# pyannote/pyannote-video

Hardware: AMD Instinct MI355X
Metric: frames/sec end-to-end detect->embed->cluster, 1080p@25fps (higher is better)
Workload: dtype f32 (detector scores, embedder) / f64 (tracker, clustering) / u8 frames; an f16 screening pass with a proven error bound decides which windows the detector's exact f32 chain is evaluated for -- results identical to dense f32 scoring (`dense_scoring`)

## Files before the change

### pyannote-video_amd/csrc/detect.hip

```cpp
#include "detect_ml.h"
#include <algorithm>
#include <thread>
#include <cmath>
#include <cstdlib>

#define RESIZE_MAXS 22
struct RowTab { int32_t top, bottom; double tb, tb1, pad; };
struct ColTab { int32_t left, pad; double lr, lr1, pad2; };

template <int RS, int NSTRIP>
__global__ void __launch_bounds__(256) resize_rows_k(const uint8_t* const* __restrict__ in_ptrs, const uint8_t* __restrict__ in_base,
                                                     size_t in_stride, int in_rb, int ih, int iw, uint8_t* __restrict__ out,
                                                     size_t out_stride, int out_rb, int oh, int ow,
                                                     const RowTab* __restrict__ rows, const ColTab* __restrict__ cols)
{
    constexpr int MAXS = (RS == 16) ? RESIZE_MAXS : (RS * 5) / 4 + 3;
    __shared__ uint32_t s_rows[4][MAXS][64];
    __shared__ uint32_t s_out[4][64];
    const int lane = threadIdx.x & 63;
    const int wave = __builtin_amdgcn_readfirstlane(threadIdx.x >> 6);
    const int c0 = blockIdx.x * 256 + wave * 64;
    const int b = blockIdx.z;
    if (c0 >= ow) return;
    const int c = min(c0 + lane, ow - 1);
    const uint8_t* in = in_ptrs ? in_ptrs[b] : in_base + (size_t)b * in_stride;
    uint8_t* ob = out + (size_t)b * out_stride + (size_t)c0 * 3;
    const ColTab ct = cols[c];
    const int left = ct.left;
    const int left0 = __builtin_amdgcn_readfirstlane(left);
    const bool has_right = (left + 1 <= iw - 1);
    const double lr = ct.lr, lr1 = ct.lr1;
    const int seg_bytes = min(ow - c0, 64) * 3;
    const bool stores = (4 * lane < seg_bytes);
    const unsigned delta = (unsigned)((uintptr_t)in & 3u);
    const __amdgpu_buffer_rsrc_t rs = __builtin_amdgcn_make_buffer_rsrc((void*)((uintptr_t)in - delta), 0, (int)(delta + (unsigned)ih * (unsigned)in_rb), 0x00020000);
    const int lane4 = 4 * lane;
    int r0 = blockIdx.y * (RS * NSTRIP), r_end = 0, s_first = 0;
    unsigned win0 = 0;
    uint32_t t[MAXS];
    auto request = [&](int q0, int& sf, unsigned& w0) {
        const int qe = min(q0 + RS, oh);
        sf = rows[q0].top;
        const int nr = rows[qe - 1].bottom - sf + 1;
        w0 = delta + (unsigned)sf * (unsigned)in_rb + 3u * (unsigned)left0;
#pragma unroll
        for (int k = 0; k < MAXS; ++k) {
            t[k] = 0;
            if (k < nr) t[k] = __builtin_amdgcn_raw_buffer_load_b32(rs, lane4, (int)((w0 + (unsigned)k * (unsigned)in_rb) & ~3u), 0);
        }
    };
    request(r0, s_first, win0);
    const uint8_t* wl = reinterpret_cast<const uint8_t*>(&s_rows[wave][0][0]) + 3 * (left - left0);
    const uint8_t* wr = wl + (has_right ? 3 : 0);
    uint8_t* so = reinterpret_cast<uint8_t*>(&s_out[wave][0]) + 3 * lane;
    const uint32_t* sd = &s_out[wave][0] + lane;
    auto hblend = [&](int srow, double* hh) {
        const int k = srow - s_first;
        const unsigned off = 256u * (unsigned)k + ((win0 + (unsigned)k * (unsigned)in_rb) & 3u);
        typedef const volatile __attribute__((address_space(3))) uint8_t* lds_bytes;
        lds_bytes pl = (lds_bytes)(wl + off);
        lds_bytes pr = (lds_bytes)(wr + off);
        const uint32_t l0 = pl[0], l1 = pl[1], l2 = pl[2], q0 = pr[0], q1 = pr[1], q2 = pr[2];
        hh[0] = lr1 * (double)l0 + lr * (double)q0;
        hh[1] = lr1 * (double)l1 + lr * (double)q1;
        hh[2] = lr1 * (double)l2 + lr * (double)q2;
    };
    const __amdgpu_buffer_rsrc_t ro = __builtin_amdgcn_make_buffer_rsrc((void*)ob, 0, (int)((unsigned)oh * (unsigned)out_rb - 3u * (unsigned)c0), 0x00020000);
    const int st_off = stores ? lane4 : 0x7fffff00;
    auto emit = [&](int r, double tb, double tb1, const double* ht, const double* hb) {
#pragma unroll
        for (int k = 0; k < 3; ++k) {
            const double v = tb1 * ht[k] + tb * hb[k];
            so[k] = (uint8_t)(v + 0.5);
        }
        __builtin_amdgcn_wave_barrier();
        const uint32_t dw = *sd;
        __builtin_amdgcn_wave_barrier();
        __builtin_amdgcn_raw_buffer_store_b32(dw, ro, st_off, r * out_rb, 0);
    };
    int r = 0, srow = 0;
    double hA[3], hB[3];
    const __attribute__((address_space(4))) RowTab* crows = (const __attribute__((address_space(4))) RowTab*)rows;
    int top_r = 0;
    auto step = [&](const double* hc, double* hn) {
        const int ra = min(r, oh - 1), rb = min(r + 1, oh - 1), rc = min(r + 2, oh - 1);
        const double tbA = crows[ra].tb, tb1A = crows[ra].tb1, tbB = crows[rb].tb, tb1B = crows[rb].tb1;
        const int topB = crows[rb].top, topC = crows[rc].top;
        hblend(min(srow + 1, ih - 1), hn);
        if (top_r == srow) {
            emit(r, tbA, tb1A, hc, hn);
            ++r;
            top_r = topB;
            if (r < r_end && top_r == srow) {
                emit(r, tbB, tb1B, hc, hn);
                ++r;
                top_r = topC;
                while (r < r_end && top_r == srow) {
                    emit(r, crows[r].tb, crows[r].tb1, hc, hn);
                    ++r;
                    top_r = crows[min(r, oh - 1)].top;
                }
            }
        }
        ++srow;
    };
#pragma unroll 1
    for (int strip = 0; strip < NSTRIP; ++strip) {
#pragma unroll
        for (int k = 0; k < MAXS; ++k) s_rows[wave][k][lane] = t[k];
        __builtin_amdgcn_wave_barrier();
        r_end = min(r0 + RS, oh);
        const int q0 = r0 + RS;
        const bool more = (strip + 1 < NSTRIP) && (q0 < oh);
        int n_first = 0;
        unsigned n_win0 = 0;
        if (more) request(q0, n_first, n_win0);
        r = r0; srow = s_first; top_r = s_first;
        hblend(srow, hA);
        while (r < r_end) {
            step(hA, hB);
            if (r >= r_end) break;
            step(hB, hA);
        }
        if (!more) break;
        __builtin_amdgcn_wave_barrier();
        r0 = q0; s_first = n_first; win0 = n_win0;
    }
}

static std::vector<double> resize_coords(int n_in, int n_out)
{
    const double scale = (n_in - 1) / (double)std::max(n_out - 1, 1);
    const char* mode = getenv("PVF_RESIZE_COORDS");
    const bool accumulate = mode && strcmp(mode, "accumulate") == 0;
    PVF_REQUIRE(!mode || accumulate || strcmp(mode, "mul") == 0, "PVF_RESIZE_COORDS must be mul or accumulate");
    std::vector<double> v((size_t)n_out);
    double a = -scale;
    for (int i = 0; i < n_out; ++i) { a += scale; v[i] = accumulate ? a : i * scale; }
    return v;
}

static void fill_row_table(std::vector<RowTab>& t, int ih, int oh)
{
    const std::vector<double> ys = resize_coords(ih, oh);
    const size_t base = t.size();
    t.resize(base + oh);
    for (int r = 0; r < oh; ++r) {
        const double y = ys[r];
        RowTab& e = t[base + r];
        e.top = (int)std::floor(y);
        e.bottom = std::min(e.top + 1, ih - 1);
        e.tb = y - e.top;
        e.tb1 = 1 - e.tb;
        e.pad = 0;
    }
}

static void fill_col_table(std::vector<ColTab>& t, int iw, int ow)
{
    const std::vector<double> xs = resize_coords(iw, ow);
    const size_t base = t.size();
    t.resize(base + ow);
    for (int c = 0; c < ow; ++c) {
        ColTab& e = t[base + c];
        e.left = (int)std::floor(xs[c]);
        e.lr = xs[c] - e.left;
        e.lr1 = 1 - e.lr;
        e.pad = 0; e.pad2 = 0;
    }
}

static void launch_resize_rows(Ctx* c, const uint8_t* const* in_ptrs, const uint8_t* in_base, size_t in_stride, int in_rb, int ih, int iw,
                               uint8_t* out, size_t out_stride, int out_rb, int oh, int ow, int batch, const RowTab* d_rows, const ColTab* d_cols)
{
    const double x_scale = (iw - 1) / (double)std::max(ow - 1, 1);
    const double y_scale = (ih - 1) / (double)std::max(oh - 1, 1);
    constexpr int RS = 16;
    PVF_REQUIRE(x_scale <= 1.25 && y_scale <= 1.25 && (RS - 1) * y_scale + 3 <= RESIZE_MAXS, "resize_rows: scale outside the pyramid's range (2x up, 6/5 down)");
    PVF_REQUIRE(out_rb % 4 == 0 && out_stride % 4 == 0 && ((uintptr_t)out & 3) == 0 && out_rb >= (ow * 3 + 3) / 4 * 4, "resize: output rows must be 4-byte aligned");
    constexpr int NSTRIP = 2;
    static const int thin = getenv("PVF_RESIZE_THIN") ? atoi(getenv("PVF_RESIZE_THIN")) : 0;
    if (thin) {
        dim3 grid8((ow + 255) / 256, (oh + 8 * NSTRIP - 1) / (8 * NSTRIP), batch);
        hipLaunchKernelGGL((resize_rows_k<8, NSTRIP>), grid8, dim3(256), 0, c->det_stream, in_ptrs, in_base, in_stride, in_rb, ih, iw, out, out_stride, out_rb, oh, ow, d_rows, d_cols);
        return;
    }
    dim3 grid((ow + 255) / 256, (oh + RS * NSTRIP - 1) / (RS * NSTRIP), batch);
    hipLaunchKernelGGL((resize_rows_k<RS, NSTRIP>), grid, dim3(256), 0, c->det_stream, in_ptrs, in_base, in_stride, in_rb, ih, iw, out, out_stride, out_rb, oh, ow, d_rows, d_cols);
}

static void pyramid_up_dims(int ih, int iw, int* oh, int* ow)
{
    const double right = ((iw - 1) + 1.25) * 2.0;
    const double bottom = ((ih - 1) + 0.75) * 2.0;
    *ow = (int)std::floor(right + 0.5) + 1;
    *oh = (int)std::floor(bottom + 0.5) + 1;
}


static inline long iround(double v) { return (long)std::floor(v + 0.5); }
static void rect_down6(long r[4]) { const double ratio = (6 - 1.0) / 6; for (int i = 0; i < 4; ++i) r[i] = iround((r[i] - 0.3) * ratio + 0.3); }
static void rect_up6(long r[4]) { const double ratio = 6 / (6 - 1.0); for (int i = 0; i < 4; ++i) r[i] = iround((r[i] - 0.3) * ratio + 0.3); }
static void rect_down2i(long r[4])
{
    r[0] = iround(r[0] / 2.0 - 1.25); r[1] = iround(r[1] / 2.0 - 0.75);
    r[2] = iround(r[2] / 2.0 - 1.25); r[3] = iround(r[3] / 2.0 - 0.75);
}
static int detector_levels(int h, int w, const DetectorModel& m)
{
    long r[4] = {0, 0, w - 1, h - 1};
    int levels = 0;
    do { rect_down6(r); ++levels; } while ((r[2] - r[0] + 1) >= m.min_w && (r[3] - r[1] + 1) >= m.min_h && levels < m.max_levels);
    return levels;
}
static void fhog_to_image(long px, long py, int cell, int pad_r, int pad_c, long* ox, long* oy)
{
    long x = (px + 1 - (pad_c - 1) / 2) * cell + 1;
    long y = (py + 1 - (pad_r - 1) / 2) * cell + 1;
    x += (x >= 0) ? cell / 2 : -(cell / 2);
    y += (y >= 0) ? cell / 2 : -(cell / 2);
    *ox = x; *oy = y;
}

struct LevelDims { int h, w; };
static std::vector<LevelDims> level_schedule(int h, int w, int upsample, const DetectorModel& m, std::vector<LevelDims>* ups)
{
    int ch = h, cw = w;
    for (int u = 0; u < upsample; ++u) {
        int nh, nw;
        pyramid_up_dims(ch, cw, &nh, &nw);
        ch = nh; cw = nw;
        if (ups) ups->push_back({ch, cw});
    }
    const int levels = detector_levels(ch, cw, m);
    std::vector<LevelDims> out;
    out.push_back({ch, cw});
    for (int l = 1; l < levels; ++l) { ch = (5 * ch) / 6; cw = (5 * cw) / 6; out.push_back({ch, cw}); }
    return out;
}

static void upload_frame_ptrs(Ctx* c, const std::vector<Frame>& frames, const uint8_t*** d_ptrs)
{
    DevBuf& d = c->s_fptr[c->det_slot & 1];
    HostBuf& h = c->h_fptr[c->det_slot & 1];
    d.ensure(frames.size() * sizeof(void*));
    h.ensure(frames.size() * sizeof(void*));
    const uint8_t** hp = h.as<const uint8_t*>();
    for (size_t i = 0; i < frames.size(); ++i) hp[i] = frames[i].d;
    HIP_CHECK(hipMemcpyAsync(d.p, hp, frames.size() * sizeof(void*), hipMemcpyHostToDevice, c->det_stream));
    *d_ptrs = d.as<const uint8_t*>();
}


__device__ __forceinline__ int ml_block(const MlStarts& st) { return (int)blockIdx.x; }
static inline int ml_grid(int total) { return total; }

__device__ __forceinline__ int ml_level(const MlStarts& st, int g)
{
    int l = 0;
    while (l + 1 < st.nl && g >= st.b0[l + 1]) ++l;
    return l;
}

#define FUSED_OUT 61
__device__ __forceinline__ uint32_t from_next_lane(uint32_t v) { return (uint32_t)__builtin_amdgcn_update_dpp(0, (int)v, 0x130, 0xf, 0xf, true); }
__device__ __forceinline__ uint32_t from_prev_lane(uint32_t v) { return (uint32_t)__builtin_amdgcn_update_dpp(0, (int)v, 0x138, 0xf, 0xf, true); }

#define FS_PAIRS 4
#define FS_COLS 65
#define FS_SLOT_DW (8 * FS_COLS * 2)
#define FS_BINS_DW (2 * 18 * 64)
#define FS_FLAG_DW (4 * 64)
#define FS_LDS_BYTES (FS_PAIRS * (FS_BINS_DW + 2 * FS_SLOT_DW + FS_FLAG_DW) * 4)
static_assert(FS_COLS * 8 == 520, "the ring's column pitch is written into the instruction strings below");
typedef __attribute__((address_space(3))) uint32_t* lds_u32;
__device__ __forceinline__ uint32_t lds_addr(const void* p) { return (uint32_t)(uintptr_t)(lds_u32)p; }

__device__ __forceinline__ void ring_write(uint32_t data_at, uint32_t flag_at, const u32x2* v, uint32_t row1)
{
    asm volatile("ds_write_b64 %0, %2\n\tds_write_b64 %0, %3 offset:520\n\tds_write_b64 %0, %4 offset:1040\n\tds_write_b64 %0, %5 offset:1560\n\t"
                 "ds_write_b64 %0, %6 offset:2080\n\tds_write_b64 %0, %7 offset:2600\n\tds_write_b64 %0, %8 offset:3120\n\t"
                 "ds_write_b64 %0, %9 offset:3640\n\tds_write_b32 %1, %10"
                 :: "v"(data_at), "v"(flag_at), "v"(v[0]), "v"(v[1]), "v"(v[2]), "v"(v[3]), "v"(v[4]), "v"(v[5]), "v"(v[6]), "v"(v[7]), "v"(row1) : "memory");
}
__device__ __forceinline__ uint32_t ring_read(uint32_t data_at, uint32_t flag_at, u32x2* own, u32x2* nb)
{
    uint32_t ready;
    asm volatile("ds_read_b32 %0, %18\n\t"
                 "ds_read_b64 %1, %17\n\tds_read_b64 %9, %17 offset:8\n\tds_read_b64 %2, %17 offset:520\n\tds_read_b64 %10, %17 offset:528\n\t"
                 "ds_read_b64 %3, %17 offset:1040\n\tds_read_b64 %11, %17 offset:1048\n\tds_read_b64 %4, %17 offset:1560\n\tds_read_b64 %12, %17 offset:1568\n\t"
                 "ds_read_b64 %5, %17 offset:2080\n\tds_read_b64 %13, %17 offset:2088\n\tds_read_b64 %6, %17 offset:2600\n\tds_read_b64 %14, %17 offset:2608\n\t"
                 "ds_read_b64 %7, %17 offset:3120\n\tds_read_b64 %15, %17 offset:3128\n\tds_read_b64 %8, %17 offset:3640\n\tds_read_b64 %16, %17 offset:3648\n\t"
                 "s_waitcnt lgkmcnt(0)"
                 : "=&v"(ready), "=&v"(own[0]), "=&v"(own[1]), "=&v"(own[2]), "=&v"(own[3]), "=&v"(own[4]), "=&v"(own[5]), "=&v"(own[6]), "=&v"(own[7]),
                   "=&v"(nb[0]), "=&v"(nb[1]), "=&v"(nb[2]), "=&v"(nb[3]), "=&v"(nb[4]), "=&v"(nb[5]), "=&v"(nb[6]), "=&v"(nb[7])
                 : "v"(data_at), "v"(flag_at) : "memory");
    return ready;
}
__device__ __forceinline__ void flag_write(uint32_t flag_at, uint32_t v)
{
    asm volatile("ds_write_b32 %0, %1" :: "v"(flag_at), "v"(v) : "memory");
}

template <int A, int B> __device__ __forceinline__ uint32_t sub_into_upper(uint32_t acc, uint32_t x, uint32_t y);
#define PVF_SUBW1(A, B)                                                                                                                  \
    template <> __device__ __forceinline__ uint32_t sub_into_upper<A, B>(uint32_t acc, uint32_t x, uint32_t y)                           \
    {                                                                                                                                    \
        asm("v_sub_u32_sdwa %0, %1, %2 dst_sel:WORD_1 dst_unused:UNUSED_PRESERVE src0_sel:BYTE_" #A " src1_sel:BYTE_" #B "\n\ts_nop 0"   \
            : "+v"(acc) : "v"(x), "v"(y));                                                                                               \
        return acc;                                                                                                                      \
    }
PVF_SUBW1(0, 0) PVF_SUBW1(1, 1) PVF_SUBW1(2, 2) PVF_SUBW1(3, 3)
#undef PVF_SUBW1
typedef short s16x2 __attribute__((ext_vector_type(2)));

template <int P>
__device__ __forceinline__ u32x2 split_grad_px(const uint32_t* up, const uint32_t* ce, const uint32_t* dn, const __amdgpu_buffer_rsrc_t& lut_rs,
                                               bool valid)
{
    uint32_t pk[3];
    int cv[3];
#define PVF_CH(K)                                                                                                                         \
    {                                                                                                                                     \
        constexpr int IU = 4 + 3 * P + K, IL = 1 + 3 * P + K, IR = 7 + 3 * P + K;                                                         \
        const uint32_t cx = ((ce[IR >> 2] >> (8 * (IR & 3))) & 0xffu) - ((ce[IL >> 2] >> (8 * (IL & 3))) & 0xffu);                          \
        pk[K] = sub_into_upper<(IU & 3), (IU & 3)>(cx, dn[IU >> 2], up[IU >> 2]);                                                          \
        const s16x2 v = __builtin_bit_cast(s16x2, pk[K]);                                                                                 \
        cv[K] = __builtin_amdgcn_sdot2(v, v, 0, false);                                                                                   \
    }
    PVF_CH(0) PVF_CH(1) PVF_CH(2)
#undef PVF_CH
    const int bv = max(cv[0], max(cv[1], cv[2]));
    const uint32_t pb = (cv[0] == bv) ? pk[0] : ((cv[1] == bv) ? pk[1] : pk[2]);
    const uint32_t off = (pb & 7u) | ((pb >> 13) & 0xff8u) | ((pb << 9) & 0x3f000u);
    u32x2 r;
    r.y = (uint32_t)__builtin_amdgcn_raw_buffer_load_b8(lut_rs, off, 0, 0);
    const float m = sqrt_exact_small((float)bv);
    r.x = valid ? __float_as_uint(m) : 0u;
    return r;
}

// ... 258 lines not shown
            sv[u] = __builtin_amdgcn_raw_buffer_load_b128(rs, tid16, 0, 0);
        }
    };
    auto fill_part = [&](float* seg, int half) {
        if ((int)threadIdx.x < SEG) {
#pragma unroll
            for (int u = 0; u < NH; ++u) {
                const int q = half * NH + u;
                uint32_t* dd = reinterpret_cast<uint32_t*>(seg + (int)threadIdx.x * PITCH + 4 * q);
                dd[0] = sv[u].x; dd[1] = sv[u].y; dd[2] = sv[u].z;
                if (q != 7) dd[3] = sv[u].w;
            }
        }
    };
    auto emit = [&](int r_out, const f32x4 (&a)[MT]) {
        const int jc = lane & 15;
        if (jc < 15) {
            const int sft = jc / 5, f = jc % 5;
            const float th = sp.thresh[f];
            const int r = r_base + r_out + FR / 2;
#pragma unroll
            for (int tt = 0; tt < MT; ++tt)
#pragma unroll
                for (int reg = 0; reg < 4; ++reg) {
                    const int pos = 4 * (lane >> 4) + reg;
                    const int cc = c_base + tt * 48 + 3 * pos + sft + FC / 2;
                    const float v = a[tt][reg];
                    if (cc < c1 && v >= th && (tt == 0 || two_tiles)) {
                        const int idx = atomicAdd(&counts[b], 1);
                        if (idx < sp.cap) {
                            CandRec rec;
                            rec.score = v - th; rec.filter = f; rec.level = l; rec.r = r; rec.c = cc;
                            cands[(size_t)b * sp.cap + idx] = rec;
                        }
                    }
                }
        }
    };
    load_part(0, 0); fill_part(s_seg, 0);
    load_part(0, 1); fill_part(s_seg, 1);
    __syncthreads();
    for (int s = 0; s < fh; ++s) {
        const float* seg = s_seg + (s & 1) * SLAB;
        float* nxt = s_seg + ((s + 1) & 1) * SLAB;
        load_part(s + 1, 0);
        const int p = (s - wave) & 1;
        const int r0 = s - p;
        bool on[R];
        bool all_on = two_tiles, any_on = false;
#pragma unroll
        for (int q = 0; q < R; ++q) {
            const int r = r0 - 2 * q;
            on[q] = (r >= 0 && r < out_rows);
            all_on = all_on && on[q];
            any_on = any_on || on[q];
        }
        if (any_on) {
            const int bop = p * NK * 2048;
            const float* a0 = seg + (3 * i) * PITCH + kq;
            u32x4 bn[R][2];
            float an[8 * MT];
#pragma unroll
            for (int q = 0; q < R; ++q) {
                bn[q][0] = __builtin_amdgcn_raw_buffer_load_b128(brs, lane16, bop + 2 * q * NK * 2048, 0);
                bn[q][1] = __builtin_amdgcn_raw_buffer_load_b128(brs, lane16, bop + 2 * q * NK * 2048 + 1024, 0);
            }
#pragma unroll
            for (int pq = 0; pq < 8; ++pq)
#pragma unroll
                for (int tt = 0; tt < MT; ++tt) an[pq * MT + tt] = a0[(tt * 48) * PITCH + 4 * pq];
#pragma unroll
            for (int n = 0; n < NK; ++n) {
                float ac[8 * MT];
                float bc[R][8];
#pragma unroll
                for (int x = 0; x < 8 * MT; ++x) ac[x] = an[x];
#pragma unroll
                for (int q = 0; q < R; ++q)
#pragma unroll
                    for (int h = 0; h < 2; ++h) {
                        const uint32_t b0 = bn[q][h].x, b1 = bn[q][h].y, b2 = bn[q][h].z, b3 = bn[q][h].w;
                        bc[q][4 * h] = __uint_as_float(b0); bc[q][4 * h + 1] = __uint_as_float(b1);
                        bc[q][4 * h + 2] = __uint_as_float(b2); bc[q][4 * h + 3] = __uint_as_float(b3);
                    }
                if (n + 1 < NK) {
#pragma unroll
                    for (int q = 0; q < R; ++q) {
                        bn[q][0] = __builtin_amdgcn_raw_buffer_load_b128(brs, lane16, bop + (2 * q * NK + n + 1) * 2048, 0);
                        bn[q][1] = __builtin_amdgcn_raw_buffer_load_b128(brs, lane16, bop + (2 * q * NK + n + 1) * 2048 + 1024, 0);
                    }
#pragma unroll
                    for (int pq = 0; pq < 8; ++pq)
#pragma unroll
                        for (int tt = 0; tt < MT; ++tt) an[pq * MT + tt] = a0[(tt * 48) * PITCH + 32 * (n + 1) + 4 * pq];
                }
                if (n == NK / 2) { fill_part(nxt, 0); load_part(s + 1, 1); }
                __builtin_amdgcn_sched_barrier(0);
                const int steps = (n == NK - 1) ? LAST_STEPS : 8;
                if (all_on) {
#pragma unroll
                    for (int pq = 0; pq < steps; ++pq)
#pragma unroll
                        for (int q = 0; q < R; ++q)
#pragma unroll
                            for (int tt = 0; tt < MT; ++tt)
                                acc[q][tt] = __builtin_amdgcn_mfma_f32_16x16x4f32(ac[pq * MT + tt], bc[q][pq], acc[q][tt], 0, 0, 0);
                } else {
#pragma unroll
                    for (int q = 0; q < R; ++q) {
                        if (!on[q]) continue;
                        if (two_tiles) {
#pragma unroll
                            for (int pq = 0; pq < steps; ++pq)
#pragma unroll
                                for (int tt = 0; tt < MT; ++tt)
                                    acc[q][tt] = __builtin_amdgcn_mfma_f32_16x16x4f32(ac[pq * MT + tt], bc[q][pq], acc[q][tt], 0, 0, 0);
                        } else {
#pragma unroll
                            for (int pq = 0; pq < steps; ++pq)
                                acc[q][0] = __builtin_amdgcn_mfma_f32_16x16x4f32(ac[pq * MT], bc[q][pq], acc[q][0], 0, 0, 0);
                        }
                    }
                }
                __builtin_amdgcn_sched_barrier(0);
            }
        }
        else { fill_part(nxt, 0); load_part(s + 1, 1); }
        if (p == 1) {
            if (on[R - 1]) emit(r0 - 2 * (R - 1), acc[R - 1]);
#pragma unroll
            for (int q = R - 1; q > 0; --q)
#pragma unroll
                for (int tt = 0; tt < MT; ++tt) acc[q][tt] = acc[q - 1][tt];
#pragma unroll
            for (int tt = 0; tt < MT; ++tt) acc[0][tt] = (f32x4){0.f, 0.f, 0.f, 0.f};
        }
        fill_part(nxt, 1);
        __syncthreads();
    }
}

struct MlPlan {
    int h = 0, w = 0, upsample = -1, B = 0;
    std::vector<LvDesc> lv;
    std::vector<LevelDims> ups;
    MlStarts feat, fused, walk;
    int feat_blocks = 0, fused_blocks = 0, walk_blocks = 0;
    size_t img_bytes = 0, feat_floats = 0, up_bytes = 0;
    LvDesc* d_lv = nullptr;
    RowTab* d_rowtab = nullptr;
    ColTab* d_coltab = nullptr;
    std::vector<size_t> up_tab, lv_tab;
    std::vector<size_t> up_ctab, lv_ctab;
    const void* ring_valid_for = nullptr;
    ScreenPlan screen;
    bool screen_built = false;
    ~MlPlan() { if (d_lv) (void)hipFree(d_lv); if (d_rowtab) (void)hipFree(d_rowtab); if (d_coltab) (void)hipFree(d_coltab); }
    MlPlan() = default;
    MlPlan(const MlPlan&) = delete;
    MlPlan& operator=(const MlPlan&) = delete;
};

struct MlPlanCache {
    std::map<std::vector<int>, std::unique_ptr<MlPlan>> plans;
    int dpp_probe = -1;
    int sqrt_probe = -1;
};
void ml_plans_free(Ctx* c)
{
    delete c->ml_plans;
    c->ml_plans = nullptr;
}

static MlPlan* ml_plan(Ctx* c, int h, int w, int upsample, int B)
{
    if (!c->ml_plans) c->ml_plans = new MlPlanCache();
    const std::vector<int> key{h, w, upsample, B};
    auto it = c->ml_plans->plans.find(key);
    if (it != c->ml_plans->plans.end()) return it->second.get();
    const DetectorModel& m = c->det;
    std::unique_ptr<MlPlan> pp(new MlPlan());
    MlPlan& p = *pp;
    p.h = h; p.w = w; p.upsample = upsample; p.B = B;
    std::vector<LevelDims> dims = level_schedule(h, w, upsample, m, &p.ups);
    PVF_REQUIRE((int)dims.size() <= ML_MAX, "too many pyramid levels");
    auto al = [](size_t v, size_t a) { return (v + a - 1) / a * a; };
    for (size_t u = 0; u + 1 < p.ups.size(); ++u) p.up_bytes = std::max(p.up_bytes, (size_t)p.ups[u].h * al((size_t)p.ups[u].w * 3, 64) * B);
    p.feat.nl = p.fused.nl = p.walk.nl = (int)dims.size();
    int chunk_big = 8;
    for (int cand : {160, 128, 96, 64, 48, 32, 24, 16}) {
        long long tasks = 0;
        for (const LevelDims& ld : dims) {
            const int hog_nr = (int)((double)ld.h / 8.0 + 0.5) - 2, hog_nc = (int)((double)ld.w / 8.0 + 0.5) - 2;
            if (hog_nr > 0 && hog_nc > 0) tasks += (long long)((hog_nc + FUSED_OUT - 1) / FUSED_OUT) * std::max(2, (hog_nr + cand - 1) / cand) * B;
        }
        if (tasks >= 2LL * c->n_cu * 2 * 4) { chunk_big = cand; break; }
    }
    if (getenv("PVF_FHOG_CHUNK") && atoi(getenv("PVF_FHOG_CHUNK")) > 0) chunk_big = atoi(getenv("PVF_FHOG_CHUNK"));
    for (size_t l = 0; l < dims.size(); ++l) {
        LvDesc d;
        memset(&d, 0, sizeof d);
        d.h = dims[l].h; d.w = dims[l].w;
        d.cells_nr = (int)((double)d.h / 8.0 + 0.5); d.cells_nc = (int)((double)d.w / 8.0 + 0.5);
        d.visible_nr = std::min(d.cells_nr * 8, d.h) - 1; d.visible_nc = std::min(d.cells_nc * 8, d.w) - 1;
        d.hog_nr = d.cells_nr - 2; d.hog_nc = d.cells_nc - 2;
        const bool feat_ok = d.hog_nr > 0 && d.hog_nc > 0;
        d.fh = feat_ok ? d.hog_nr + m.frows - 1 : 0; d.fw = feat_ok ? d.hog_nc + m.fcols - 1 : 0;
        d.valid_score = (d.fh >= m.frows && d.fw >= m.fcols) ? 1 : 0;
        d.rb = (int)al((size_t)d.w * 3, 64);
        d.img_off = (long long)p.img_bytes; d.img_stride = (long long)d.h * d.rb;
        p.img_bytes += (size_t)d.img_stride * B;
        d.fwp = feat_ok ? d.fw + FEAT_PAD_COLS : 0;
        d.feat_off = (long long)p.feat_floats; d.feat_stride = (long long)d.fh * d.fwp * PVF_FHOG_STRIDE;
        p.feat_floats += (size_t)d.feat_stride * B;
        d.feat_bx = feat_ok ? (d.fwp + 255) / 256 : 0;
        const int out_c = d.fw - 9;
        d.score_bx = d.valid_score ? (out_c + 95) / 96 : 0;
        d.strips = feat_ok ? (d.hog_nc + FUSED_OUT - 1) / FUSED_OUT : 0;
        {
            const int nch = std::max(2, (d.hog_nr + chunk_big - 1) / chunk_big);
            d.chunk_rows = std::max((d.hog_nr + nch - 1) / nch, 1);
        }
        d.chunks = feat_ok ? (d.hog_nr + d.chunk_rows - 1) / d.chunk_rows : 0;
        d.fused_tasks = d.strips * d.chunks * B;
        p.feat.b0[l] = p.feat_blocks; p.feat_blocks += d.feat_bx * d.fh * B;
        p.fused.b0[l] = p.fused_blocks; p.fused_blocks += (d.fused_tasks + 3) / 4;
        p.lv.push_back(d);
    }
    const int nl = (int)dims.size();
    {
        long long total = 0;
        for (const LvDesc& d : p.lv) if (d.valid_score) total += (long long)d.score_bx * (d.fh - 9 + 9) * B;
        const int slots = 4 * 256;
        int roll_max = (int)std::max<long long>(64, total / slots / 2);
        if (getenv("PVF_SCORE_SEG")) roll_max = std::max(2, atoi(getenv("PVF_SCORE_SEG")));
        for (int l = 0; l < nl; ++l) {
            LvDesc& d = p.lv[l];
            const int out_r = d.fh - 9;
            d.roll_nseg = d.valid_score ? (out_r + roll_max - 1) / roll_max : 0;
            d.roll_rows = d.valid_score ? ((out_r + d.roll_nseg - 1) / d.roll_nseg + 1) / 2 * 2 : 0;
            if (d.valid_score) d.roll_nseg = (out_r + d.roll_rows - 1) / d.roll_rows;
            p.walk.b0[l] = p.walk_blocks; p.walk_blocks += d.score_bx * d.roll_nseg * B;
        }
    }
    p.feat.b0[nl] = p.feat_blocks; p.walk.b0[nl] = p.walk_blocks;
    p.fused.b0[nl] = p.fused_blocks;
    HIP_CHECK(hipMalloc((void**)&p.d_lv, sizeof(LvDesc) * nl));
    HIP_CHECK(hipMemcpy(p.d_lv, p.lv.data(), sizeof(LvDesc) * nl, hipMemcpyHostToDevice));
    {
        std::vector<RowTab> tab;
        int ch = h;
        for (size_t u = 0; u < p.ups.size(); ++u) { p.up_tab.push_back(tab.size()); fill_row_table(tab, ch, p.ups[u].h); ch = p.ups[u].h; }
        p.lv_tab.push_back(0);
        for (int l = 1; l < nl; ++l) { p.lv_tab.push_back(tab.size()); fill_row_table(tab, p.lv[l - 1].h, p.lv[l].h); }
        HIP_CHECK(hipMalloc((void**)&p.d_rowtab, sizeof(RowTab) * std::max<size_t>(tab.size(), 1)));
        if (!tab.empty()) HIP_CHECK(hipMemcpy(p.d_rowtab, tab.data(), sizeof(RowTab) * tab.size(), hipMemcpyHostToDevice));
        std::vector<ColTab> ctab;
        int cw2 = w;
        for (size_t u = 0; u < p.ups.size(); ++u) { p.up_ctab.push_back(ctab.size()); fill_col_table(ctab, cw2, p.ups[u].w); cw2 = p.ups[u].w; }
        p.lv_ctab.push_back(0);
        for (int l = 1; l < nl; ++l) { p.lv_ctab.push_back(ctab.size()); fill_col_table(ctab, p.lv[l - 1].w, p.lv[l].w); }
        HIP_CHECK(hipMalloc((void**)&p.d_coltab, sizeof(ColTab) * std::max<size_t>(ctab.size(), 1)));
        if (!ctab.empty()) HIP_CHECK(hipMemcpy(p.d_coltab, ctab.data(), sizeof(ColTab) * ctab.size(), hipMemcpyHostToDevice));
    }
    MlPlan* raw = pp.get();
    c->ml_plans->plans[key] = std::move(pp);
    return raw;
}

static MlPlan* ml_build_pyramid(Ctx* c, const std::vector<Frame>& frames, int upsample)
{
    const int B = (int)frames.size();
    const int h = frames[0].h, w = frames[0].w;
    for (auto& f : frames) PVF_REQUIRE(f.h == h && f.w == w, "batched frames must share one size");
    MlPlan* p = ml_plan(c, h, w, upsample, B);
    c->s_pyr.ensure(p->img_bytes + p->up_bytes + 256);
    uint8_t* base = c->s_pyr.as<uint8_t>();
    uint8_t* up_tmp = base + ((p->img_bytes + 63) / 64) * 64;
    const uint8_t** d_ptrs = nullptr;
    upload_frame_ptrs(c, frames, &d_ptrs);
    ProfScope ps(c, "pyramid", c->det_stream);
    auto al = [](size_t v, size_t a) { return (v + a - 1) / a * a; };
    const uint8_t* cur = nullptr;
    int ch = h, cw = w, crb = w * 3;
    size_t cstride = 0;
    for (size_t u = 0; u < p->ups.size(); ++u) {
        const bool last = (u + 1 == p->ups.size());
        uint8_t* dst = last ? base + p->lv[0].img_off : up_tmp;
        const int drb = (int)al((size_t)p->ups[u].w * 3, 64);
        const size_t dstride = (size_t)p->ups[u].h * drb;
        launch_resize_rows(c, cur ? nullptr : d_ptrs, cur, cstride, crb, ch, cw, dst, dstride, drb, p->ups[u].h, p->ups[u].w, B, p->d_rowtab + p->up_tab[u], p->d_coltab + p->up_ctab[u]);
        cur = dst; cstride = dstride; crb = drb; ch = p->ups[u].h; cw = p->ups[u].w;
    }
    if (!cur) {
        for (int b = 0; b < B; ++b)
            HIP_CHECK(hipMemcpy2DAsync(base + p->lv[0].img_off + (size_t)b * p->lv[0].img_stride, (size_t)p->lv[0].rb, frames[b].d, (size_t)w * 3,
                                       (size_t)w * 3, (size_t)h, hipMemcpyDeviceToDevice, c->det_stream));
    }
    for (size_t l = 1; l < p->lv.size(); ++l)
        launch_resize_rows(c, nullptr, base + p->lv[l - 1].img_off, (size_t)p->lv[l - 1].img_stride, p->lv[l - 1].rb, p->lv[l - 1].h, p->lv[l - 1].w,
                           base + p->lv[l].img_off, (size_t)p->lv[l].img_stride, p->lv[l].rb, p->lv[l].h, p->lv[l].w, B, p->d_rowtab + p->lv_tab[l], p->d_coltab + p->lv_ctab[l]);
    return p;
}

__global__ void dpp_probe_k(int* out)
{
    const int lane = threadIdx.x;
    out[lane] = (int)from_next_lane((uint32_t)(lane + 100));
    out[64 + lane] = (int)from_prev_lane((uint32_t)(lane + 100));
}
#define SQRT_PROBE_N (2 * 255 * 255 + 1)
__global__ void sqrt_probe_k(float* out)
{
    const int i = blockIdx.x * blockDim.x + threadIdx.x;
    if (i < SQRT_PROBE_N) out[i] = sqrt_exact_small((float)i);
}
static void check_dpp_direction(Ctx* c)
{
    MlPlanCache* pc = c->ml_plans;
    if (pc->dpp_probe < 0) {
        int* d = nullptr;
        HIP_CHECK(hipMalloc((void**)&d, 128 * sizeof(int) + SQRT_PROBE_N * sizeof(float)));
        float* ds = reinterpret_cast<float*>(d + 128);
        hipLaunchKernelGGL(dpp_probe_k, dim3(1), dim3(64), 0, c->det_stream, d);
        hipLaunchKernelGGL(sqrt_probe_k, dim3((SQRT_PROBE_N + 255) / 256), dim3(256), 0, c->det_stream, ds);
        int h[128];
        std::vector<float> hs(SQRT_PROBE_N);
        HIP_CHECK(hipMemcpyAsync(h, d, sizeof h, hipMemcpyDeviceToHost, c->det_stream));
        HIP_CHECK(hipMemcpyAsync(hs.data(), ds, SQRT_PROBE_N * sizeof(float), hipMemcpyDeviceToHost, c->det_stream));
        HIP_CHECK(hipStreamSynchronize(c->det_stream));
        (void)hipFree(d);
        bool ok = true;
        for (int i = 0; i < 64; ++i) {
            ok = ok && h[i] == (i < 63 ? i + 101 : 0);
            ok = ok && h[64 + i] == (i > 0 ? i + 99 : 0);
        }
        pc->dpp_probe = ok ? 1 : 0;
        bool sq = true;
        for (int i = 0; i < SQRT_PROBE_N; ++i) sq = sq && hs[i] == (float)std::sqrt((double)i);
        pc->sqrt_probe = sq ? 1 : 0;
    }
    PVF_REQUIRE(pc->dpp_probe == 1, "v_mov_b32_dpp wave_shl / wave_shr do not move data as the FHOG kernel expects on this device");
    PVF_REQUIRE(pc->sqrt_probe == 1, "v_sqrt_f32 is not within one step below the correctly rounded root on this device: the FHOG kernel's one-sided correction does not hold");
}

static MlPlan* ml_features(Ctx* c, const std::vector<Frame>& frames, int upsample)
{
    const DetectorModel& m = c->det;
    const int B = (int)frames.size();
    MlPlan* p = ml_build_pyramid(c, frames, upsample);
    const int oy = (m.frows - 1) / 2, ox = (m.fcols - 1) / 2;
    const void* feat_before = c->s_feat.p;
    c->s_feat.ensure(p->feat_floats * sizeof(float) + 64);
    if (p->fused_blocks == 0) return p;
    check_dpp_direction(c);
    ProfScope ps(c, "fhog", c->det_stream);
    if (c->s_feat.p != feat_before || c->feat_ring_owner != (const void*)p) {
        hipLaunchKernelGGL(feat_ring_zero_k, dim3(ml_grid(p->feat_blocks)), dim3(256), 0, c->det_stream, p->feat, p->d_lv, B, c->s_feat.as<float>(), oy, ox);
        c->feat_ring_owner = (const void*)p;
    }
    static std::atomic<uint64_t> attr_set{0};
    const uint64_t bit = 1ull << (c->device & 63);
    if (!(attr_set.load() & bit)) {
        HIP_CHECK(hipFuncSetAttribute(reinterpret_cast<const void*>(fhog_split_ml_k), hipFuncAttributeMaxDynamicSharedMemorySize, FS_LDS_BYTES));
        attr_set.fetch_or(bit);
    }
    hipLaunchKernelGGL(fhog_split_ml_k, dim3(ml_grid(p->fused_blocks)), dim3(512), FS_LDS_BYTES, c->det_stream, p->fused, p->d_lv, B,
                       c->s_pyr.as<uint8_t>(), c->s_feat.as<float>(), orientation_lut_wrapped(c), oy, ox);
    return p;
}

static void det_run_batch_ml(Ctx* c, const std::vector<Frame>& frames, int upsample, const ScoreParams& sp0, int* d_counts, CandRec* d_cands)
{
    const DetectorModel& m = c->det;
    const int B = (int)frames.size();
    MlPlan* p = ml_features(c, frames, upsample);
    if (p->walk_blocks == 0) return;
    if (c->det_screen && !c->det_screen_suspended) {
        if (!p->screen_built) { screen_plan_build(p->screen, p->lv, B); p->screen_built = true; }
        if (p->screen.usable) {
            ProfScope ps(c, "score_screened", c->det_stream);
            screen_launch(c, p->screen, p->d_lv, B, c->s_feat.as<float>(), sp0, d_counts, d_cands, d_counts + B);
            ++c->screen_batches;
            return;
        }
    }
    ProfScope ps(c, "score", c->det_stream);
    const size_t lds = (size_t)2 * (((2 * 48 + 11) * 31 + 3) / 4 * 4) * sizeof(float);
    const float4* b4 = reinterpret_cast<const float4*>(m.d_bmfma4);
    hipLaunchKernelGGL(score_roll_k, dim3(p->walk_blocks), dim3(128), lds, c->det_stream, p->walk, p->d_lv, B, c->s_feat.as<float>(), b4, sp0, d_counts, d_cands);
}

void det_pyramid_level(Ctx* c, const Frame& f, int upsample, int level, std::vector<uint8_t>* out, int* oh, int* ow)
{
    PVF_REQUIRE(c->det.loaded, "detector not loaded");
    std::vector<Frame> fr{f};
    MlPlan* p = ml_build_pyramid(c, fr, upsample);
    PVF_REQUIRE(level >= 0 && level < (int)p->lv.size(), "pyramid level out of range");
    *oh = p->lv[level].h; *ow = p->lv[level].w;
    if (out) {
        out->resize((size_t)(*oh) * (*ow) * 3);
        HIP_CHECK(hipMemcpy2DAsync(out->data(), (size_t)(*ow) * 3, c->s_pyr.as<uint8_t>() + p->lv[level].img_off, (size_t)p->lv[level].rb,
                                   (size_t)(*ow) * 3, (size_t)(*oh), hipMemcpyDeviceToHost, c->det_stream));
    }
    HIP_CHECK(hipStreamSynchronize(c->det_stream));
}

void det_pyramid_batch(Ctx* c, const std::vector<Frame>& frames, int upsample)
{
    PVF_REQUIRE(c->det.loaded, "detector not loaded");
    PVF_REQUIRE(!frames.empty(), "pyramid batch: no frames");
    (void)ml_build_pyramid(c, frames, upsample);
    HIP_CHECK(hipStreamSynchronize(c->det_stream));
}

void det_level_features(Ctx* c, const Frame& f, int upsample, int level, std::vector<float>* out, int* fh, int* fw)
{
    PVF_REQUIRE(c->det.loaded, "detector not loaded");
    std::vector<Frame> fr{f};
    MlPlan* p = ml_features(c, fr, upsample);
    PVF_REQUIRE(level >= 0 && level < (int)p->lv.size(), "pyramid level out of range");
    const LvDesc& d = p->lv[level];
    *fh = d.fh; *fw = d.fw;
    if (out) {
        out->resize((size_t)d.fh * d.fw * PVF_FHOG_STRIDE);
        std::vector<float> dev((size_t)d.feat_stride);
        if (!dev.empty())
            HIP_CHECK(hipMemcpyAsync(dev.data(), c->s_feat.as<float>() + d.feat_off, dev.size() * sizeof(float), hipMemcpyDeviceToHost, c->det_stream));
        HIP_CHECK(hipStreamSynchronize(c->det_stream));
        for (int y = 0; y < d.fh; ++y)
            for (int j = 0; j < 8; ++j)
                for (int x = 0; x < d.fw; ++x)
                    memcpy(out->data() + ((size_t)y * d.fw + x) * PVF_FHOG_STRIDE + 4 * j, dev.data() + feat_at(y, j, x, d.fwp), 4 * sizeof(float));
    }
    HIP_CHECK(hipStreamSynchronize(c->det_stream));
}

static bool raw_less(const RawDet& x, const RawDet& y)
{
    if (x.score != y.score) return x.score > y.score;
    if (x.filter != y.filter) return x.filter < y.filter;
    if (x.level != y.level) return x.level < y.level;
    if (x.r != y.r) return x.r < y.r;
    return x.c < y.c;
}

static void decode_candidates(const DetectorModel& m, int upsample, const CandRec* q, int n, std::vector<RawDet>& v);

static void screen_verdict(Ctx* c, const int* ctl)
{
    if (!c->det_screen || c->det_screen_suspended) return;
    c->screen_listed += std::min(ctl[SCR_FLAGGED], c->screen_list_cap);
    if (ctl[SCR_FLAGGED] > c->screen_list_cap || ctl[SCR_VIOLATION] != 0) {
        HIP_CHECK(hipStreamSynchronize(c->det_stream));
// ... 165 lines not shown
```

Baseline: 4471.

## Resize pyramid in f32 with exact f64 fallback for near-tie rows

The bilinear pyramid resize now runs in single precision by default. Each output value is checked for being near a rounding boundary, and any row where a lane is near a tie is recomputed in f64 after the strip. The aim is to replace costly f64 arithmetic while keeping byte-identical output. Pixel gathers now use aligned LDS word loads with alignbyte instead of three volatile byte loads. This adds a ballot per row, a deferred redo loop, and float weights stored in the table padding.

Measured after the change: 4502 (median of 5 runs). About the same (+0.7%).

```diff
diff --git a/pyannote-video_amd/csrc/detect.hip b/pyannote-video_amd/csrc/detect.hip
--- a/pyannote-video_amd/csrc/detect.hip
+++ b/pyannote-video_amd/csrc/detect.hip
@@ -3,12 +3,23 @@
 #include <thread>
 #include <cmath>
 #include <cstdlib>
+#include <type_traits>
 
 #define RESIZE_MAXS 22
-struct RowTab { int32_t top, bottom; double tb, tb1, pad; };
-struct ColTab { int32_t left, pad; double lr, lr1, pad2; };
-
-template <int RS, int NSTRIP>
+struct RowTab { int32_t top, bottom; double tb, tb1; float tbf, tb1f; };
+struct ColTab { int32_t left, pad; double lr, lr1; float lrf, lr1f; };
+static_assert(sizeof(RowTab) == 32 && sizeof(ColTab) == 32, "resize tables: one 32-byte entry per row / column");
+
+enum { RESIZE_F64 = 0, RESIZE_F32 = 1, RESIZE_FALLBACK = 2 };
+__device__ __forceinline__ double resize_h64(double lr1, double lr, uint32_t l, uint32_t q) { return lr1 * (double)l + lr * (double)q; }
+__device__ __forceinline__ uint8_t resize_v64(double tb1, double tb, double ht, double hb)
+{
+    const double v = tb1 * ht + tb * hb;
+    return (uint8_t)(v + 0.5);
+}
+#define RESIZE_EPS (1.0f / 8192.0f)
+
+template <int RS, int NSTRIP, int ARITH>
 __global__ void __launch_bounds__(256) resize_rows_k(const uint8_t* const* __restrict__ in_ptrs, const uint8_t* __restrict__ in_base,
                                                      size_t in_stride, int in_rb, int ih, int iw, uint8_t* __restrict__ out,
                                                      size_t out_stride, int out_rb, int oh, int ow,
@@ -30,6 +41,8 @@
     const int left0 = __builtin_amdgcn_readfirstlane(left);
     const bool has_right = (left + 1 <= iw - 1);
     const double lr = ct.lr, lr1 = ct.lr1;
+    const float lrf = ct.lrf, lr1f = ct.lr1f;
+    using HT = typename std::conditional<ARITH == RESIZE_F64, double, float>::type;
     const int seg_bytes = min(ow - c0, 64) * 3;
     const bool stores = (4 * lane < seg_bytes);
     const unsigned delta = (unsigned)((uintptr_t)in & 3u);
@@ -54,37 +67,93 @@
     const uint8_t* wr = wl + (has_right ? 3 : 0);
     uint8_t* so = reinterpret_cast<uint8_t*>(&s_out[wave][0]) + 3 * lane;
     const uint32_t* sd = &s_out[wave][0] + lane;
-    auto hblend = [&](int srow, double* hh) {
+    auto hblend64 = [&](int srow, double* hh) {
         const int k = srow - s_first;
         const unsigned off = 256u * (unsigned)k + ((win0 + (unsigned)k * (unsigned)in_rb) & 3u);
         typedef const volatile __attribute__((address_space(3))) uint8_t* lds_bytes;
         lds_bytes pl = (lds_bytes)(wl + off);
         lds_bytes pr = (lds_bytes)(wr + off);
         const uint32_t l0 = pl[0], l1 = pl[1], l2 = pl[2], q0 = pr[0], q1 = pr[1], q2 = pr[2];
-        hh[0] = lr1 * (double)l0 + lr * (double)q0;
-        hh[1] = lr1 * (double)l1 + lr * (double)q1;
-        hh[2] = lr1 * (double)l2 + lr * (double)q2;
+        hh[0] = resize_h64(lr1, lr, l0, q0);
+        hh[1] = resize_h64(lr1, lr, l1, q1);
+        hh[2] = resize_h64(lr1, lr, l2, q2);
+    };
+    const unsigned wlo = (unsigned)(3 * (left - left0)), wro = wlo + (has_right ? 3u : 0u);
+    typedef const __attribute__((address_space(3))) uint32_t* lds_words;
+    const unsigned sbase = (unsigned)(size_t)(const __attribute__((address_space(3))) uint32_t*)&s_rows[wave][0][0];
+    auto pixel = [&](unsigned boff) -> uint32_t {
+        const unsigned a = sbase + boff;
+        lds_words pw = (lds_words)(size_t)(a & ~3u);
+        return __builtin_amdgcn_alignbyte(pw[1], pw[0], a);
+    };
+    auto hblend = [&](int srow, HT* hh) {
+        if constexpr (ARITH == RESIZE_F64) {
+            hblend64(srow, hh);
+        } else {
+            const int k = srow - s_first;
+            const unsigned off = 256u * (unsigned)k + ((win0 + (unsigned)k * (unsigned)in_rb) & 3u);
+            const uint32_t L = pixel(wlo + off), Q = pixel(wro + off);
+            hh[0] = fmaf(lr1f, (float)(L & 0xffu), lrf * (float)(Q & 0xffu));
+            hh[1] = fmaf(lr1f, (float)((L >> 8) & 0xffu), lrf * (float)((Q >> 8) & 0xffu));
+            hh[2] = fmaf(lr1f, (float)((L >> 16) & 0xffu), lrf * (float)((Q >> 16) & 0xffu));
+        }
     };
     const __amdgpu_buffer_rsrc_t ro = __builtin_amdgcn_make_buffer_rsrc((void*)ob, 0, (int)((unsigned)oh * (unsigned)out_rb - 3u * (unsigned)c0), 0x00020000);
     const int st_off = stores ? lane4 : 0x7fffff00;
-    auto emit = [&](int r, double tb, double tb1, const double* ht, const double* hb) {
-#pragma unroll
-        for (int k = 0; k < 3; ++k) {
-            const double v = tb1 * ht[k] + tb * hb[k];
-            so[k] = (uint8_t)(v + 0.5);
+    const __attribute__((address_space(4))) RowTab* crows = (const __attribute__((address_space(4))) RowTab*)rows;
+    uint32_t fix = 0;
+    int row_off = st_off;
+    auto emit = [&](int r, HT tb, HT tb1, const HT* ht, const HT* hb) {
+        if constexpr (ARITH == RESIZE_F64) {
+#pragma unroll
+            for (int k = 0; k < 3; ++k) so[k] = resize_v64(tb1, tb, ht[k], hb[k]);
+        } else {
+            uint32_t u[3];
+            bool near = (ARITH == RESIZE_FALLBACK);
+#pragma unroll
+            for (int k = 0; k < 3; ++k) {
+                const float w = fmaf(tb1, ht[k], fmaf(tb, hb[k], 0.5f));
+                u[k] = (uint32_t)w;
+                near |= fabsf(__builtin_amdgcn_fractf(w) - 0.5f) > 0.5f - RESIZE_EPS;
+            }
+            const bool redo = __builtin_amdgcn_ballot_w64(near) != 0;
+            fix |= redo ? 1u << (r - r0) : 0u;
+            row_off = redo ? 0x7fffff00 : st_off;
+#pragma unroll
+            for (int k = 0; k < 3; ++k) so[k] = (uint8_t)u[k];
         }
         __builtin_amdgcn_wave_barrier();
         const uint32_t dw = *sd;
         __builtin_amdgcn_wave_barrier();
-        __builtin_amdgcn_raw_buffer_store_b32(dw, ro, st_off, r * out_rb, 0);
+        __builtin_amdgcn_raw_buffer_store_b32(dw, ro, row_off, r * out_rb, 0);
+    };
+    auto redo_rows = [&]() {
+        while (fix) {
+            const int rr = r0 + __builtin_ctz(fix);
+            fix &= fix - 1;
+            double dt[3], db[3];
+            hblend64(crows[rr].top, dt);
+            hblend64(crows[rr].bottom, db);
+            const double tb64 = crows[rr].tb, tb164 = crows[rr].tb1;
+#pragma unroll
+            for (int k = 0; k < 3; ++k) so[k] = resize_v64(tb164, tb64, dt[k], db[k]);
+            __builtin_amdgcn_wave_barrier();
+            const uint32_t dw = *sd;
+            __builtin_amdgcn_wave_barrier();
+            __builtin_amdgcn_raw_buffer_store_b32(dw, ro, st_off, rr * out_rb, 0);
+        }
     };
     int r = 0, srow = 0;
-    double hA[3], hB[3];
-    const __attribute__((address_space(4))) RowTab* crows = (const __attribute__((address_space(4))) RowTab*)rows;
+    HT hA[3], hB[3];
     int top_r = 0;
-    auto step = [&](const double* hc, double* hn) {
+    auto wts = [&](int q, HT& tb, HT& tb1) {
+        if constexpr (ARITH == RESIZE_F64) { tb = crows[q].tb; tb1 = crows[q].tb1; }
+        else { tb = crows[q].tbf; tb1 = crows[q].tb1f; }
+    };
+    auto step = [&](const HT* hc, HT* hn) {
         const int ra = min(r, oh - 1), rb = min(r + 1, oh - 1), rc = min(r + 2, oh - 1);
-        const double tbA = crows[ra].tb, tb1A = crows[ra].tb1, tbB = crows[rb].tb, tb1B = crows[rb].tb1;
+        HT tbA, tb1A, tbB, tb1B;
+        wts(ra, tbA, tb1A); wts(rb, tbB, tb1B);
         const int topB = crows[rb].top, topC = crows[rc].top;
         hblend(min(srow + 1, ih - 1), hn);
         if (top_r == srow) {
@@ -96,7 +165,9 @@
                 ++r;
                 top_r = topC;
                 while (r < r_end && top_r == srow) {
-                    emit(r, crows[r].tb, crows[r].tb1, hc, hn);
+                    HT tbC, tb1C;
+                    wts(r, tbC, tb1C);
+                    emit(r, tbC, tb1C, hc, hn);
                     ++r;
                     top_r = crows[min(r, oh - 1)].top;
                 }
@@ -122,6 +193,7 @@
             if (r >= r_end) break;
             step(hB, hA);
         }
+        if constexpr (ARITH != RESIZE_F64) redo_rows();
         if (!more) break;
         __builtin_amdgcn_wave_barrier();
         r0 = q0; s_first = n_first; win0 = n_win0;
@@ -152,7 +224,8 @@
         e.bottom = std::min(e.top + 1, ih - 1);
         e.tb = y - e.top;
         e.tb1 = 1 - e.tb;
-        e.pad = 0;
+        e.tbf = (float)e.tb;
+        e.tb1f = (float)e.tb1;
     }
 }
 
@@ -166,12 +239,36 @@
         e.left = (int)std::floor(xs[c]);
         e.lr = xs[c] - e.left;
         e.lr1 = 1 - e.lr;
-        e.pad = 0; e.pad2 = 0;
-    }
+        e.lrf = (float)e.lr;
+        e.lr1f = (float)e.lr1;
+        e.pad = 0;
+    }
+}
+
+static int resize_arith_mode()
+{
+    const char* mode = getenv("PVF_RESIZE_ARITH");
+    if (!mode || strcmp(mode, "f32") == 0) return RESIZE_F32;
+    if (strcmp(mode, "f64") == 0) return RESIZE_F64;
+    PVF_REQUIRE(strcmp(mode, "fallback") == 0, "PVF_RESIZE_ARITH must be f32, f64 or fallback");
+    return RESIZE_FALLBACK;
+}
+
+template <int RS, int NSTRIP>
+static void launch_resize_k(Ctx* c, dim3 grid, int arith, const uint8_t* const* in_ptrs, const uint8_t* in_base, size_t in_stride, int in_rb, int ih,
+                            int iw, uint8_t* out, size_t out_stride, int out_rb, int oh, int ow, const RowTab* d_rows, const ColTab* d_cols)
+{
+    if (arith == RESIZE_F64)
+        hipLaunchKernelGGL((resize_rows_k<RS, NSTRIP, RESIZE_F64>), grid, dim3(256), 0, c->det_stream, in_ptrs, in_base, in_stride, in_rb, ih, iw, out, out_stride, out_rb, oh, ow, d_rows, d_cols);
+    else if (arith == RESIZE_F32)
+        hipLaunchKernelGGL((resize_rows_k<RS, NSTRIP, RESIZE_F32>), grid, dim3(256), 0, c->det_stream, in_ptrs, in_base, in_stride, in_rb, ih, iw, out, out_stride, out_rb, oh, ow, d_rows, d_cols);
+    else
+        hipLaunchKernelGGL((resize_rows_k<RS, NSTRIP, RESIZE_FALLBACK>), grid, dim3(256), 0, c->det_stream, in_ptrs, in_base, in_stride, in_rb, ih, iw, out, out_stride, out_rb, oh, ow, d_rows, d_cols);
 }
 
 static void launch_resize_rows(Ctx* c, const uint8_t* const* in_ptrs, const uint8_t* in_base, size_t in_stride, int in_rb, int ih, int iw,
-                               uint8_t* out, size_t out_stride, int out_rb, int oh, int ow, int batch, const RowTab* d_rows, const ColTab* d_cols)
+                               uint8_t* out, size_t out_stride, int out_rb, int oh, int ow, int batch, const RowTab* d_rows, const ColTab* d_cols,
+                               int arith)
 {
     const double x_scale = (iw - 1) / (double)std::max(ow - 1, 1);
     const double y_scale = (ih - 1) / (double)std::max(oh - 1, 1);
@@ -182,11 +279,11 @@
     static const int thin = getenv("PVF_RESIZE_THIN") ? atoi(getenv("PVF_RESIZE_THIN")) : 0;
     if (thin) {
         dim3 grid8((ow + 255) / 256, (oh + 8 * NSTRIP - 1) / (8 * NSTRIP), batch);
-        hipLaunchKernelGGL((resize_rows_k<8, NSTRIP>), grid8, dim3(256), 0, c->det_stream, in_ptrs, in_base, in_stride, in_rb, ih, iw, out, out_stride, out_rb, oh, ow, d_rows, d_cols);
+        launch_resize_k<8, NSTRIP>(c, grid8, arith, in_ptrs, in_base, in_stride, in_rb, ih, iw, out, out_stride, out_rb, oh, ow, d_rows, d_cols);
         return;
     }
     dim3 grid((ow + 255) / 256, (oh + RS * NSTRIP - 1) / (RS * NSTRIP), batch);
-    hipLaunchKernelGGL((resize_rows_k<RS, NSTRIP>), grid, dim3(256), 0, c->det_stream, in_ptrs, in_base, in_stride, in_rb, ih, iw, out, out_stride, out_rb, oh, ow, d_rows, d_cols);
+    launch_resize_k<RS, NSTRIP>(c, grid, arith, in_ptrs, in_base, in_stride, in_rb, ih, iw, out, out_stride, out_rb, oh, ow, d_rows, d_cols);
 }
 
 static void pyramid_up_dims(int ih, int iw, int* oh, int* ow)
@@ -751,6 +848,7 @@
     ColTab* d_coltab = nullptr;
     std::vector<size_t> up_tab, lv_tab;
     std::vector<size_t> up_ctab, lv_ctab;
+    int resize_arith = RESIZE_F32;
     const void* ring_valid_for = nullptr;
     ScreenPlan screen;
     bool screen_built = false;
@@ -846,6 +944,7 @@
     p.fused.b0[nl] = p.fused_blocks;
     HIP_CHECK(hipMalloc((void**)&p.d_lv, sizeof(LvDesc) * nl));
     HIP_CHECK(hipMemcpy(p.d_lv, p.lv.data(), sizeof(LvDesc) * nl, hipMemcpyHostToDevice));
+    p.resize_arith = resize_arith_mode();
     {
         std::vector<RowTab> tab;
         int ch = h;
@@ -888,7 +987,7 @@
         uint8_t* dst = last ? base + p->lv[0].img_off : up_tmp;
         const int drb = (int)al((size_t)p->ups[u].w * 3, 64);
         const size_t dstride = (size_t)p->ups[u].h * drb;
-        launch_resize_rows(c, cur ? nullptr : d_ptrs, cur, cstride, crb, ch, cw, dst, dstride, drb, p->ups[u].h, p->ups[u].w, B, p->d_rowtab + p->up_tab[u], p->d_coltab + p->up_ctab[u]);
+        launch_resize_rows(c, cur ? nullptr : d_ptrs, cur, cstride, crb, ch, cw, dst, dstride, drb, p->ups[u].h, p->ups[u].w, B, p->d_rowtab + p->up_tab[u], p->d_coltab + p->up_ctab[u], p->resize_arith);
         cur = dst; cstride = dstride; crb = drb; ch = p->ups[u].h; cw = p->ups[u].w;
     }
     if (!cur) {
@@ -898,7 +997,7 @@
     }
     for (size_t l = 1; l < p->lv.size(); ++l)
         launch_resize_rows(c, nullptr, base + p->lv[l - 1].img_off, (size_t)p->lv[l - 1].img_stride, p->lv[l - 1].rb, p->lv[l - 1].h, p->lv[l - 1].w,
-                           base + p->lv[l].img_off, (size_t)p->lv[l].img_stride, p->lv[l].rb, p->lv[l].h, p->lv[l].w, B, p->d_rowtab + p->lv_tab[l], p->d_coltab + p->lv_ctab[l]);
+                           base + p->lv[l].img_off, (size_t)p->lv[l].img_stride, p->lv[l].rb, p->lv[l].h, p->lv[l].w, B, p->d_rowtab + p->lv_tab[l], p->d_coltab + p->lv_ctab[l], p->resize_arith);
     return p;
 }
 
```
